# tsy935/eeg-gnn-ssl

Measured on AMD Instinct MI355X. Metric: EEG clips/sec (60s, 19ch, K=2, 2-layer x64) fwd+bwd, higher is better.
Workload: dtype f32

## Files before the change

### eeg_gnn_ssl_amd/csrc/api.cpp

```cpp
#include <atomic>
#include <cmath>
#include <cstdarg>
#include <cstdio>
#include <cstring>

#include <string>
#include <vector>

#include "../../include/eeg_dcrnn.h"
#include "../../include/eeg_dcrnn_dev.h"
#include "../../include/eeg_dcrnn_prof.h"
#include "kernels_decoder.h"
#include "kernels_diffuse.h"
#include "kernels_data.h"
#include "kernels_feat.h"
#include "kernels_gemm.h"
#include "kernels_gemm_bf.h"
#include "kernels_graph.h"
#include "kernels_head.h"
#include "kernels_pack.h"
#include "spec_common.h"
#include "spec_launch.h"
#include "kernels_tail.h"
#include "prof.h"
// ... 555 lines not shown
    if (p == nullptr) return fail("zero: null pointer");
    if (reinterpret_cast<uintptr_t>(p) % 16 != 0)
        return hipMemsetAsync(p, 0, bytes, S_(stream)) == hipSuccess ? 0 : fail("zero: memset failed");
    const size_t n16 = bytes / 16;
    const int blocks = (int)(n16 / 256 < 1 ? 1 : (n16 / 256 > 1024 ? 1024 : n16 / 256));
    EEG_LAUNCH_P("zero", zero_kernel, dim3(blocks), dim3(256), 0, S_(stream), reinterpret_cast<float4*>(p), n16,
                 reinterpret_cast<unsigned char*>(p) + 16 * n16, (int)(bytes - 16 * n16));
    return check_launch("zero");
}

int eeg_dcrnn_hop_polys(const float* const* supports, int n_supports, int n_graphs, int N, int K, float* P_out,
                        void* stream) {
    if (n_supports < 1 || n_supports > 4) return fail("hop_polys: n_supports=%d unsupported (1..4)", n_supports);
    if (N < 1 || N > kMaxNodes) return fail("hop_polys: num_nodes=%d unsupported", N);
    if (K < 0) return fail("hop_polys: max_diffusion_step=%d unsupported (>= 0)", K);
    if (n_graphs < 1) return fail("hop_polys: no graphs (n_graphs=%d)", n_graphs);
    if (K == 0) return 0;
    if (n_supports * K + 1 > kMaxM) return fail("hop_polys: %d supports x K=%d exceeds %d hop matrices", n_supports, K, kMaxM);
    SupPtrs sp;
    for (int i = 0; i < 4; ++i) sp.p[i] = i < n_supports ? supports[i] : nullptr;
    const size_t lds = 4 * kMaxNodes * kMaxNodes * sizeof(float);
    EEG_LAUNCH_P("hop_polys", hop_polys_kernel, dim3(n_graphs), dim3(round_up(N * N, 64)), lds, S_(stream), sp, n_supports, N, K, P_out);
    return check_launch("hop_polys");
}

size_t eeg_dcrnn_pack_floats(int Fin, int H, int M) { return make_cell_pack(Fin, H, M).total; }

int eeg_dcrnn_pack_cell(const float* Wg, const float* bg, const float* Wc, const float* bc, int Fin, int H, int M,
                        float* pack, void* stream) {
    if (!seq_h_supported(H)) return fail("pack_cell: rnn_units=%d unsupported", H);
    if (Fin < 4 || Fin % 4 != 0) return fail("pack_cell: input dim %d must be a positive multiple of 4", Fin);
    if (!seq_m_supported(M)) return fail("pack_cell: num hop matrices M=%d unsupported (1,2,3,4,5,7)", M);
    CellPack p = make_cell_pack(Fin, H, M);
    EEG_LAUNCH_P("pack_cell", pack_cell_kernel, dim3(512), dim3(256), 0, S_(stream), Wg, bg, Wc, bc, pack, p);
    return check_launch("pack_cell");
}
size_t eeg_dcrnn_pack3_halves(int Fin, int H, int M) { return pack3_supported(Fin, H, M) ? make_pack3(Fin, H, M).total : 0; }
int eeg_dcrnn_pack_cell_bf16x3(const float* Wg, const float* Wc, int Fin, int H, int M, uint16_t* pack3, void* stream) {
    if (!pack3_supported(Fin, H, M)) return fail("pack_cell_bf16x3: rnn_units=%d, input_dim=%d, %d hop matrices: the bf16 split exists for 64 units", H, Fin, M);
    if (Wg == nullptr || Wc == nullptr || pack3 == nullptr) return fail("pack_cell_bf16x3: null pointer");
    EEG_LAUNCH_P("pack_cell", pack_cell_bf3_kernel, dim3(512), dim3(256), 0, S_(stream), Wg, Wc, Fin, H, M, pack3);
    return check_launch("pack_cell_bf3");
}

int eeg_dcrnn_diffuse_fwd(const float* X, const float* P, int p_batched, int S, int B, int N, int F, int M,
                          float* planes, void* stream) {
    if (N < 1 || N > kMaxNodes || F < 4 || F % 4 != 0 || M < 1 || M > kMaxM) return fail("diffuse_fwd: bad dims N=%d F=%d M=%d", N, F, M);
    if (S < 1 || B < 1) return fail("diffuse_fwd: empty input (S=%d, B=%d)", S, B);
    return diffuse_fwd(X, P, p_batched, S, B, N, F, M, planes, S_(stream));
}
int eeg_dcrnn_diffuse_adj(const float* Z, const float* P, int p_batched, int S, int B, int N, int F, int M,
                          float* dX, void* stream) {
    if (N < 1 || N > kMaxNodes || F < 4 || F % 4 != 0 || M < 1 || M > kMaxM) return fail("diffuse_adj: bad dims N=%d F=%d M=%d", N, F, M);
    if (S < 1 || B < 1) return fail("diffuse_adj: empty input (S=%d, B=%d)", S, B);
    return diffuse_adj(Z, P, p_batched, S, B, N, F, M, dX, S_(stream));
}

static bool layer_dims_positive(const eeg_layer_dims* d) {
    return d != nullptr && d->T >= 1 && d->B >= 1 && d->N >= 1 && d->H >= 1 && d->Fin >= 1 && d->M >= 1;
}
size_t eeg_dcrnn_layer_fwd_ws_floats(const eeg_layer_dims* d) {
    if (!layer_dims_positive(d)) return 0;
    const size_t xw = (size_t)d->T * d->B * d->N * 3 * d->H;
    return d->spectral != nullptr ? xw + (size_t)d->N * spec_rows(d->T * d->B) * 3 * d->H : xw;
}

size_t eeg_dcrnn_spectral_basis_floats(int N) { return (N >= 1 && N <= kMaxNodes) ? (size_t)spec_basis_floats(N) : 0; }
// ... 1071 lines not shown
```

### eeg_gnn_ssl_amd/csrc/kernels_pack.h

```cpp
#pragma once
#include "common.h"
#include "nnq_order.h"
#include "spec_common.h"
#include "pack_cell.h"

namespace eeg {

__global__ void pack_cell_kernel(const float* __restrict__ Wg, const float* __restrict__ bg,
                                 const float* __restrict__ Wc, const float* __restrict__ bc,
                                 float* __restrict__ out, CellPack p) {
    pack_cell_body(Wg, bg, Wc, bc, out, p, (int)blockIdx.x, (int)gridDim.x);
}

__global__ void pack_dense_kernel(const float* __restrict__ W, int F, int M, int O, float* __restrict__ out) {
    const size_t total = (size_t)F * M * O;
    const int nct = O / 16;
    for (size_t e = (size_t)blockIdx.x * blockDim.x + threadIdx.x; e < total; e += (size_t)gridDim.x * blockDim.x) {
        const int lane = e & 63, ct = (e >> 6) % nct, ks = (e >> 6) / nct;
        const int k = 4 * ks + (lane >> 4), j = 16 * ct + (lane & 15);
        const int m = k / F, f = k % F;
        out[e] = W[((size_t)f * M + m) * O + j];
    }
}

// ... 49 lines not shown
    const float sv[4] = {sum.x, sum.y, sum.z, sum.w};
    const bool accumulate = (kind_flags & 8) != 0;
    const int kind = kind_flags & 7;
#pragma unroll
    for (int e = 0; e < 4; ++e) {
        const size_t idx = idx4 + e;
        const int k = idx / O, o = idx % O;
        float* dst;
        if (kind == 0) {
            const int m = k / Fin, f = k % Fin;
            dst = o < 2 * H ? &dWg[((size_t)f * M + m) * (2 * H) + o] : &dWc[((size_t)f * M + m) * H + (o - 2 * H)];
        } else if (kind == 1) {
            dst = &dWg[((size_t)(Fin + k % H) * M + k / H) * (2 * H) + o];
        } else if (kind == 3) {
            dst = &dWg[idx];
        } else if (kind == 4) {
            dst = &dWg[((size_t)(k % Fin) * M + k / Fin) * O + o];
        } else {
            dst = &dWc[((size_t)(Fin + k % H) * M + k / H) * H + o];
        }
        *dst = accumulate ? *dst + sv[e] : sv[e];
    }
}
__global__ __launch_bounds__(256) void reduce_unpack_kernel(const float* __restrict__ part, int nsplit, int K, int O,
                                                            int kind_flags, int Fin, int H, int M,
                                                            float* __restrict__ dWg, float* __restrict__ dWc) {
    reduce_unpack_block(blockIdx.x, part, nsplit, K, O, kind_flags, Fin, H, M, dWg, dWc);
}
__device__ __forceinline__ void reduce_bias_block(int blk, float* sm, const float* __restrict__ part, int B, int H,
                                                  float* __restrict__ dbg, float* __restrict__ dbc) {
    const int c = threadIdx.x & 15, q = threadIdx.x >> 4;
    const int j = blk * 16 + c;
    float s = 0.f;
    if (j < 3 * H)
        for (int b = q; b < B; b += 16) s += part[(size_t)b * 3 * H + j];
    sm[q * 16 + c] = s;
    __syncthreads();
    if (q == 0 && j < 3 * H) {
        float t = 0.f;
        for (int i = 0; i < 16; ++i) t += sm[i * 16 + c];
        if (j < 2 * H) dbg[j] = t; else dbc[j - 2 * H] = t;
    }
}
struct ReduceJobs {
    const float* part[3]; int nsplit[3]; int K[3]; int O[3]; int nblocks[3];
    const float* bias_part; int bias_B; float* dbg; float* dbc;
};
__global__ __launch_bounds__(256) void reduce_unpack3_kernel(ReduceJobs jobs, int flags, int Fin, int H, int M,
                                                             float* __restrict__ dWg, float* __restrict__ dWc) {
    int b = blockIdx.x, j = 0;
    if (b >= jobs.nblocks[0]) { b -= jobs.nblocks[0]; j = 1; }
    if (j == 1 && b >= jobs.nblocks[1]) { b -= jobs.nblocks[1]; j = 2; }
    if (j == 2 && b >= jobs.nblocks[2]) {
        EEG_DYN_SMEM(sm);
        reduce_bias_block(b - jobs.nblocks[2], sm, jobs.bias_part, jobs.bias_B, H, jobs.dbg, jobs.dbc);
        return;
    }
    reduce_unpack_block(b, jobs.part[j], jobs.nsplit[j], jobs.K[j], jobs.O[j], j | flags, Fin, H, M, dWg, dWc);
}

__global__ __launch_bounds__(256) void reduce_unpack3s_kernel(ReduceJobs jobs, SpecFoldJobs sj, int flags, int Fin, int H, int M,
                                                              float* __restrict__ dWg, float* __restrict__ dWc) {
    int b = blockIdx.x;
#pragma unroll
    for (int k = 0; k < 3; ++k) {
        if (sj.j[k].part == nullptr) continue;
        if (b < sj.j[k].nblocks) {
            spec_fold_block(b, sj.j[k], k, sj.basis, sj.N, (flags & 8) != 0 ? 1 : 0, Fin, H, M, dWg, dWc);
            return;
        }
        b -= sj.j[k].nblocks;
    }
#pragma unroll
    for (int j = 1; j < 3; ++j) {
        if (sj.j[j].part != nullptr) continue;
        if (b < jobs.nblocks[j]) {
            reduce_unpack_block(b, jobs.part[j], jobs.nsplit[j], jobs.K[j], jobs.O[j], j | flags, Fin, H, M, dWg, dWc);
            return;
        }
        b -= jobs.nblocks[j];
    }
    EEG_DYN_SMEM(sm);
    reduce_bias_block(b, sm, jobs.bias_part, jobs.bias_B, H, jobs.dbg, jobs.dbc);
}

__global__ void colsum_partial_kernel(const float* __restrict__ A, int R, int C, int rpc, float* __restrict__ partial) {
    EEG_DYN_SMEM(sm);
    const int c = threadIdx.x & 127, q = threadIdx.x >> 7;
    const int col = blockIdx.y * 128 + c;
    const int r0 = blockIdx.x * rpc, r1 = (r0 + rpc < R) ? r0 + rpc : R;
    float a0 = 0.f, a1 = 0.f, a2 = 0.f, a3 = 0.f;
    if (col < C) {
        int r = r0 + q;
        for (; r + 6 < r1; r += 8) {
// ... 101 lines not shown
```

### eeg_gnn_ssl_amd/csrc/kernels_spectral.h

```cpp
#pragma once
#include "spec_common.h"
#include "spec_launch.h"

namespace eeg {

__global__ __launch_bounds__(256) void spectral_basis_kernel(const float* __restrict__ S, int N, float* __restrict__ out) {
    EEG_DYN_SMEM(sm);
    double* A = reinterpret_cast<double*>(sm);
    double* V = A + 32 * 32;
    double* cs = V + 32 * 32;
    int* pq = reinterpret_cast<int*>(cs + 32);
    double* red = reinterpret_cast<double*>(pq + 32);
    const int tid = threadIdx.x;
    const int NP = (N + 1) & ~1, NH = NP / 2;
    for (int e = tid; e < 32 * 32; e += 256) {
        const int i = e >> 5, j = e & 31;
        A[e] = (i < N && j < N) ? 0.5 * ((double)S[i * N + j] + (double)S[j * N + i]) : 0.0;
        V[e] = i == j ? 1.0 : 0.0;
    }
    __syncthreads();
    for (int sweep = 0; sweep < kSpecSweeps; ++sweep) {
        for (int r = 0; r < NP - 1; ++r) {
            if (tid < NH) {
                int p = tid == 0 ? NP - 1 : (r + tid) % (NP - 1);
                int q = tid == 0 ? r : (r - tid + (NP - 1)) % (NP - 1);
                if (p > q) { const int t = p; p = q; q = t; }
                double c = 1.0, s = 0.0;
                if (q < N) {
                    const double apq = A[p * 32 + q];
                    if (fabs(apq) > 1e-300) {
                        const double theta = (A[q * 32 + q] - A[p * 32 + p]) / (2.0 * apq);
                        const double t = (theta >= 0.0 ? 1.0 : -1.0) / (fabs(theta) + sqrt(theta * theta + 1.0));
                        c = 1.0 / sqrt(t * t + 1.0);
                        s = t * c;
// ... 36 lines not shown
            t = m == 0 ? t0 : t1;
            for (int k = 2; k <= m; ++k) { t = 2.0 * lam * t1 - t0; t0 = t1; t1 = t; }
        }
        out[N * N + e] = (float)t;
    }
    double rmax = 0.0, omax = 0.0, smax = 0.0;
    for (int e = tid; e < N * N; e += 256) {
        const int i = e / N, j = e % N;
        double rec = 0.0;
        for (int k = 0; k < N; ++k) rec += V[i * 32 + k] * A[k * 32 + k] * V[j * 32 + k];
        rmax = fmax(rmax, fabs((double)S[e] - rec));
        if (i != j) omax = fmax(omax, fabs(A[i * 32 + j]));
        smax = fmax(smax, fabs((double)S[e]));
    }
    for (int which = 0; which < 3; ++which) {
        __syncthreads();
        red[tid] = which == 0 ? rmax : (which == 1 ? omax : smax);
        __syncthreads();
        if (tid == 0) {
            double m = 0.0;
            for (int i = 0; i < 256; ++i) m = fmax(m, red[i]);
            out[N * N + kSpecTc + which] = (float)m;
        }
    }
    if (tid >= 3 && tid < kSpecInfo) out[N * N + kSpecTc + tid] = 0.f;
    if (tid < 32) {
        double c = 0.0;
        if (tid < N)
            for (int n = 0; n < N; ++n) c += V[n * 32 + tid];
        out[N * N + kSpecTc + kSpecInfo + tid] = (float)c;
    }
}

__device__ __forceinline__ void pack_spectral_body(const float* __restrict__ Wg, const float* __restrict__ Wc, const float* __restrict__ basis,
                                                   float* __restrict__ out, const SpecPack& p, int bid, int nb) {
    const int Fin = p.Fin, H = p.H, M = p.M, N = p.N;
    const float* tc = basis + N * N;
    const NnqOrder ox = make_nnq_order(1, Fin), ot = make_nnq_order(1, 3 * H);
    const size_t stride = (size_t)nb * blockDim.x;
    for (size_t idx = (size_t)bid * blockDim.x + threadIdx.x; idx < p.total; idx += stride) {
        if (idx >= p.sxr) {
            const size_t e0 = idx - p.sxr;
            const int i = (int)(e0 / p.sxr_stride), e = (int)(e0 - (size_t)i * p.sxr_stride), f = e / (3 * H), o = e - f * 3 * H;
            float v = 0.f;
            if (f < Fin)
                for (int m = 0; m < M; ++m) {
                    const float w = o < 2 * H ? Wg[((size_t)f * M + m) * (2 * H) + o] : Wc[((size_t)f * M + m) * H + (o - 2 * H)];
                    v = fmaf(tc[m * 32 + i], w, v);
                }
            out[idx] = v;
            continue;
        }
        const bool tr = idx >= p.sxtq;
        const size_t bs = tr ? p.sxtq_stride : p.sxq_stride, e0 = idx - (tr ? p.sxtq : p.sxq);
        const int i = (int)(e0 / bs);
        const size_t e = e0 - (size_t)i * bs;
        const int s4 = e & 3, lane = (e >> 2) & 63, nct = tr ? p.nct_t : p.nct_x;
        const int ct = (int)((e >> 8) % nct), c = (int)((e >> 8) / nct), j = 16 * ct + (lane & 15);
        const int k = nnq_k_of(tr ? ot : ox, c, lane >> 4, s4);
        float v = 0.f;
        if (k >= 0) {
            const int f = tr ? j : k, o = tr ? k : j;
            if (f < Fin) {
                for (int m = 0; m < M; ++m) {
                    const float w = o < 2 * H ? Wg[((size_t)f * M + m) * (2 * H) + o] : Wc[((size_t)f * M + m) * H + (o - 2 * H)];
                    v = fmaf(tc[m * 32 + i], w, v);
                }
            }
        }
        out[idx] = v;
    }
}
__global__ void pack_spectral_kernel(const float* __restrict__ Wg, const float* __restrict__ Wc, const float* __restrict__ basis,
                                     float* __restrict__ out, SpecPack p) {
    pack_spectral_body(Wg, Wc, basis, out, p, (int)blockIdx.x, (int)gridDim.x);
}

__device__ __forceinline__ size_t spec_sample(size_t r, int map, int T, int B) { return map ? (r % B) * (size_t)T + r / B : r; }

template <int N>
__global__ __launch_bounds__(256) void spec_mix_in_kernel(const float* __restrict__ X, const float* __restrict__ basis, int S, int Sp,
                                                         int F, int map, int T, int B, float* __restrict__ Xh) {
    const int F4 = F / 4, SPW = blockDim.x / F4;
    const int tl = threadIdx.x / F4, c4 = threadIdx.x % F4;
    if (tl >= SPW) return;
    const float* __restrict__ U = basis;
    const float4* X4 = reinterpret_cast<const float4*>(X);
    float4* O4 = reinterpret_cast<float4*>(Xh);
    for (int r = blockIdx.x * SPW + tl; r < Sp; r += gridDim.x * SPW) {
        if (r >= S) {
#pragma unroll
            for (int i = 0; i < N; ++i) O4[((size_t)i * Sp + r) * F4 + c4] = make_float4(0.f, 0.f, 0.f, 0.f);
            continue;
        }
        const size_t s = spec_sample((size_t)r, map, T, B);
        float4 x[N];
#pragma unroll
        for (int n = 0; n < N; ++n) x[n] = X4[(s * N + n) * F4 + c4];
#pragma unroll
        for (int i = 0; i < N; ++i) {
            float4 a = make_float4(0.f, 0.f, 0.f, 0.f);
#pragma unroll
            for (int n = 0; n < N; ++n) {
// ... 133 lines not shown
```

### eeg_gnn_ssl_amd/csrc/pack_cell.h

```cpp
#pragma once
#include "common.h"
#include "nnq_order.h"

namespace eeg {

struct CellPack {
    int Fin, H, M;
    size_t bx;
    size_t bias;
    size_t bhg;
    size_t bhc;
    size_t b1;
    size_t b2;
    size_t bxt;
    size_t c1;
    size_t c2;
    size_t bxq;
    size_t bxtq;
    bool has_bxq, has_bxtq;
    size_t total;
};

__host__ __device__ inline CellPack make_cell_pack(int Fin, int H, int M) {
    CellPack p;
    p.Fin = Fin; p.H = H; p.M = M;
    size_t o = 0;
    p.bx = o;   o += (size_t)M * Fin * 3 * H;
    p.bias = o; o += (size_t)round_up(3 * H, 64);
    p.bhg = o;  o += (size_t)M * H * 2 * H;
    p.bhc = o;  o += (size_t)M * H * H;
    p.b1 = o;   o += (size_t)M * H * H;
    p.b2 = o;   o += (size_t)M * 2 * H * H;
    p.bxt = o;  o += (size_t)3 * H * round_up(M * Fin, 16);
    p.c1 = o;   o += (size_t)M * H * cell_pack_cx_cols(Fin, H);
    p.c2 = o;   o += (size_t)M * 2 * H * cell_pack_cx_cols(Fin, H);
    p.has_bxq = (3 * H) % 192 == 0;
    p.has_bxtq = (M * Fin) % 192 == 0 && (3 * H) % 4 == 0 && make_nnq_order(1, 3 * H).ntail <= 2;
    p.bxq = o;  o += p.has_bxq ? (size_t)round_up(make_nnq_order(M, Fin).nch, 4) * (3 * H / 16) * 256 : 0;
    p.bxtq = o; o += p.has_bxtq ? (size_t)make_nnq_order(1, 3 * H).nch * (M * Fin / 16) * 256 : 0;
    p.total = o;
    return p;
}

__device__ __forceinline__ float ref_wg(const float* Wg, int M, int H, int f_all, int m, int o) {
    return Wg[((size_t)f_all * M + m) * (2 * H) + o];
}
__device__ __forceinline__ float ref_wc(const float* Wc, int M, int H, int f_all, int m, int o) {
    return Wc[((size_t)f_all * M + m) * H + o];
}

__device__ __forceinline__ void pack_cell_body(const float* __restrict__ Wg, const float* __restrict__ bg,
                                               const float* __restrict__ Wc, const float* __restrict__ bc,
                                               float* __restrict__ out, const CellPack& p, int bid, int nb) {
    const int Fin = p.Fin, H = p.H, M = p.M;
    const size_t stride = (size_t)nb * blockDim.x;
    for (size_t idx = (size_t)bid * blockDim.x + threadIdx.x; idx < p.total; idx += stride) {
        float v = 0.f;
        if (idx < p.bias) {
            const size_t e = idx - p.bx;
            const int lane = e & 63, nct = 3 * H / 16;
            const int ct = (e >> 6) % nct, ks = (e >> 6) / nct;
            const int k = 4 * ks + (lane >> 4), j = 16 * ct + (lane & 15);
            const int m = k / Fin, f = k % Fin;
            v = j < 2 * H ? ref_wg(Wg, M, H, f, m, j) : ref_wc(Wc, M, H, f, m, j - 2 * H);
        } else if (idx < p.bhg) {
            const int j = idx - p.bias;
            v = j < 2 * H ? bg[j] : (j < 3 * H ? bc[j - 2 * H] : 0.f);
        } else if (idx < p.bhc) {
            const size_t e = idx - p.bhg;
            const int lane = e & 63, nct = 2 * H / 16;
            const int ct = (e >> 6) % nct, ks = (e >> 6) / nct;
            const int k = kperm(ks, lane >> 4), j = 16 * ct + (lane & 15);
            v = ref_wg(Wg, M, H, Fin + k % H, k / H, j);
        } else if (idx < p.b1) {
            const size_t e = idx - p.bhc;
            const int lane = e & 63, nct = H / 16;
            const int ct = (e >> 6) % nct, ks = (e >> 6) / nct;
            const int k = kperm(ks, lane >> 4), j = 16 * ct + (lane & 15);
            v = ref_wc(Wc, M, H, Fin + k % H, k / H, j);
        } else if (idx < p.b2) {
            const size_t e = idx - p.b1;
            const int lane = e & 63, nct = H / 16;
            const int ct = (e >> 6) % nct, ks = (e >> 6) / nct;
            const int k = kperm(ks, lane >> 4), f = 16 * ct + (lane & 15);
            v = ref_wc(Wc, M, H, Fin + f, k / H, k % H);
        } else if (idx < p.bxt) {
            const size_t e = idx - p.b2;
            const int lane = e & 63, nct = H / 16;
            const int ct = (e >> 6) % nct, ks = (e >> 6) / nct;
            const int k = kperm(ks, lane >> 4), f = 16 * ct + (lane & 15);
            v = ref_wg(Wg, M, H, Fin + f, k / (2 * H), k % (2 * H));
        } else if (idx < p.c1) {
            const size_t e = idx - p.bxt;
            const int lane = e & 63, nct = round_up(M * Fin, 16) / 16;
            const int ct = (e >> 6) % nct, ks = (e >> 6) / nct;
            const int o = 4 * ks + (lane >> 4), j = 16 * ct + (lane & 15);
            if (j < M * Fin) {
                const int m = j / Fin, f = j % Fin;
                v = o < 2 * H ? ref_wg(Wg, M, H, f, m, o) : ref_wc(Wc, M, H, f, m, o - 2 * H);
            }
        } else if (idx >= p.bxq) {
            const bool tr = idx >= p.bxtq;
            const size_t e = idx - (tr ? p.bxtq : p.bxq);
            const int s4 = e & 3, lane = (e >> 2) & 63, nct = tr ? M * Fin / 16 : 3 * H / 16;
            const int ct = (e >> 8) % nct, c = (e >> 8) / nct, j = 16 * ct + (lane & 15);
            const int k = nnq_k_of(tr ? make_nnq_order(1, 3 * H) : make_nnq_order(M, Fin), c, lane >> 4, s4);
            if (k >= 0) {
                if (!tr) {
                    const int m = k / Fin, f = k % Fin;
                    v = j < 2 * H ? ref_wg(Wg, M, H, f, m, j) : ref_wc(Wc, M, H, f, m, j - 2 * H);
                } else {
                    const int m = j / Fin, f = j % Fin;
                    v = k < 2 * H ? ref_wg(Wg, M, H, f, m, k) : ref_wc(Wc, M, H, f, m, k - 2 * H);
                }
            }
        } else {
            const bool gate = idx >= p.c2;
            const size_t e = idx - (gate ? p.c2 : p.c1);
            const int lane = e & 63, nct = cell_pack_cx_cols(Fin, H) / 16, W = gate ? 2 * H : H;
            const int ct = (e >> 6) % nct, ks = (e >> 6) / nct;
            const int k = kperm(ks, lane >> 4), j = 16 * ct + (lane & 15);
            const int f_all = j < H ? Fin + j : j - H;
            if (j < H + Fin) v = gate ? ref_wg(Wg, M, H, f_all, k / W, k % W) : ref_wc(Wc, M, H, f_all, k / W, k % W);
        }
        out[idx] = v;
    }
}
}
```

### eeg_gnn_ssl_amd/csrc/spec_common.h

```cpp
#pragma once
#include "common.h"
#include "nnq_order.h"

namespace eeg {

constexpr int kSpecTc = kMaxM * 32, kSpecInfo = 32, kSpecCsum = 32;
__host__ __device__ constexpr int spec_basis_floats(int N) { return N * N + kSpecTc + kSpecInfo + kSpecCsum; }
__host__ __device__ constexpr int spec_csum_offset(int N) { return N * N + kSpecTc + kSpecInfo; }
__host__ __device__ constexpr int spec_rows(int S) { return round_up(S, 16); }
constexpr int kSpecSweeps = 12;

struct SpecPack {
    int Fin, H, M, N;
    int nch_x, nct_x, nch_t, nct_t;
    size_t sxq, sxq_stride, sxtq, sxtq_stride, sxr, sxr_stride, total;
};
__host__ __device__ inline SpecPack make_spec_pack(int Fin, int H, int M, int N) {
    SpecPack p;
    p.Fin = Fin; p.H = H; p.M = M; p.N = N;
    p.nch_x = make_nnq_order(1, Fin).nch; p.nct_x = 3 * H / 16;
    p.nch_t = make_nnq_order(1, 3 * H).nch; p.nct_t = round_up(Fin, 16) / 16;
    p.sxq_stride = (size_t)p.nch_x * p.nct_x * 256;
    p.sxtq_stride = (size_t)p.nch_t * p.nct_t * 256;
    p.sxq = 0;
    p.sxtq = p.sxq + p.sxq_stride * N;
    p.sxr = p.sxtq + p.sxtq_stride * N;
    p.sxr_stride = (size_t)round_up(Fin, 8) * 3 * H;
    p.total = p.sxr + p.sxr_stride * N;
    return p;
}
struct SpecFoldJob {
    const float* part;
    int spg, K, O, nblocks;
};
struct SpecFoldJobs {
    SpecFoldJob j[3];
    const float* basis;
    int N;
};
__host__ __device__ inline size_t spec_fold_lds_bytes(int M, int nsplit_max) { return 256 * 16 + (size_t)M * nsplit_max * sizeof(float); }
template <int MM>
__device__ __forceinline__ void spec_fold_block_m(int block, const SpecFoldJob& jb, int kind, const float* __restrict__ basis, int N,
                                                   int acc_flag, int Fin, int H, int M, float* __restrict__ dWg, float* __restrict__ dWc) {
    EEG_DYN_SMEM(sm);
    float4 (*red)[16] = reinterpret_cast<float4 (*)[16]>(sm);
    float* tcl = sm + 256 * 4;
    const int O = jb.O;
    const size_t total = (size_t)jb.K * O;
    const int g = threadIdx.x >> 4, q = threadIdx.x & 15;
    const size_t idx4 = ((size_t)block * 16 + q) * 4;
    const float* tc = basis + N * N;
    const int nsplit = N * jb.spg;
    for (int e = threadIdx.x; e < M * nsplit; e += 256) {
        const int m = e / nsplit, sp = e - m * nsplit;
        tcl[e] = tc[m * 32 + sp / jb.spg];
    }
    __syncthreads();
    float4 a[MM];
#pragma unroll
    for (int m = 0; m < MM; ++m) a[m] = make_float4(0.f, 0.f, 0.f, 0.f);
    if (idx4 < total) {
        constexpr int UN = 8;
        for (int base = g; base < nsplit; base += 16 * UN) {
            float4 v[UN];
#pragma unroll
            for (int u = 0; u < UN; ++u) {
                const int sp = base + 16 * u;
                v[u] = sp < nsplit ? *reinterpret_cast<const float4*>(jb.part + (size_t)sp * total + idx4) : make_float4(0.f, 0.f, 0.f, 0.f);
            }
#pragma unroll
            for (int u = 0; u < UN; ++u) {
                const int sp = base + 16 * u < nsplit ? base + 16 * u : 0;
#pragma unroll
                for (int m = 0; m < MM; ++m) {
                    if (m < M) {
                        const float t = tcl[m * nsplit + sp];
                        a[m].x = fmaf(t, v[u].x, a[m].x); a[m].y = fmaf(t, v[u].y, a[m].y);
                        a[m].z = fmaf(t, v[u].z, a[m].z); a[m].w = fmaf(t, v[u].w, a[m].w);
                    }
                }
            }
        }
    }
#pragma unroll
    for (int m = 0; m < MM; ++m) {
        if (m >= M) break;
        __syncthreads();
        red[g][q] = a[m];
        __syncthreads();
        if (g == 0 && idx4 < total) {
            float4 sum = red[0][q];
#pragma unroll
            for (int u = 1; u < 16; ++u) {
                const float4 v = red[u][q];
                sum.x += v.x; sum.y += v.y; sum.z += v.z; sum.w += v.w;
            }
            const float sv[4] = {sum.x, sum.y, sum.z, sum.w};
#pragma unroll
            for (int e = 0; e < 4; ++e) {
                const size_t idx = idx4 + e;
                const int f = (int)(idx / O), o = (int)(idx % O);
                float* dst;
                if (kind == 0) dst = o < 2 * H ? &dWg[((size_t)f * M + m) * (2 * H) + o] : &dWc[((size_t)f * M + m) * H + (o - 2 * H)];
                else if (kind == 1) dst = &dWg[((size_t)(Fin + f) * M + m) * (2 * H) + o];
                else dst = &dWc[((size_t)(Fin + f) * M + m) * H + o];
                *dst = acc_flag ? *dst + sv[e] : sv[e];
            }
        }
    }
}
__device__ __forceinline__ void spec_fold_block(int block, const SpecFoldJob& jb, int kind, const float* __restrict__ basis, int N,
                                                int acc_flag, int Fin, int H, int M, float* __restrict__ dWg, float* __restrict__ dWc) {
    if (M <= 4) spec_fold_block_m<4>(block, jb, kind, basis, N, acc_flag, Fin, H, M, dWg, dWc);
    else spec_fold_block_m<kMaxM>(block, jb, kind, basis, N, acc_flag, Fin, H, M, dWg, dWc);
}

}
```

### eeg_gnn_ssl_amd/csrc/spec_inst.cpp

```cpp
#include "kernels_gemm_g.h"
#include "kernels_gemm_f.h"
#include "kernels_spectral.h"
#include "pack_cell.h"
#include "spec_launch.h"
#include "prof.h"

namespace eeg {

constexpr int kMaxPackJobs = 8;
struct PackJob {
    const float *Wg, *bg, *Wc, *bc, *basis;
    float* out;
    int spectral;
    CellPack cp;
    SpecPack sp;
};
struct PackJobs { PackJob j[kMaxPackJobs]; };
__global__ void pack_cells_kernel(PackJobs jobs) {
    const PackJob& jb = jobs.j[blockIdx.y];
    if (jb.spectral) pack_spectral_body(jb.Wg, jb.Wc, jb.basis, jb.out, jb.sp, (int)blockIdx.x, (int)gridDim.x);
    else pack_cell_body(jb.Wg, jb.bg, jb.Wc, jb.bc, jb.out, jb.cp, (int)blockIdx.x, (int)gridDim.x);
}


size_t spec_pack_floats(int Fin, int H, int M, int N) { return make_spec_pack(Fin, H, M, N).total; }

int launch_spec_basis(const float* S, int N, float* basis, hipStream_t st) {
    EEG_SET_MAX_LDS(spectral_basis_kernel, kSpecBasisLds);
    EEG_LAUNCH_P("spec_basis", spectral_basis_kernel, dim3(1), dim3(256), kSpecBasisLds, st, S, N, basis);
    return hipGetLastError() == hipSuccess ? 0 : 2;
}

int launch_spec_pack(const float* Wg, const float* Wc, const float* basis, int Fin, int H, int M, int N, float* spack, hipStream_t st) {
    const SpecPack p = make_spec_pack(Fin, H, M, N);
    EEG_LAUNCH_P("pack_cell", pack_spectral_kernel, dim3(1024), dim3(256), 0, st, Wg, Wc, basis, spack, p);
    return hipGetLastError() == hipSuccess ? 0 : 2;
}

int launch_pack_cells(int n_cells, const float* const* Wg, const float* const* bg, const float* const* Wc, const float* const* bc,
                      const int* Fin, int H, int M, float* const* packs, const float* basis, int N, float* const* spacks, hipStream_t st) {
    PackJobs jobs{};
    int n = 0;
    for (int c = 0; c < n_cells; ++c) {
        if (n + (spacks != nullptr ? 2 : 1) > kMaxPackJobs) return 1;
        PackJob& a = jobs.j[n++];
        a.Wg = Wg[c]; a.bg = bg[c]; a.Wc = Wc[c]; a.bc = bc[c]; a.basis = nullptr; a.out = packs[c]; a.spectral = 0;
        a.cp = make_cell_pack(Fin[c], H, M);
        if (spacks != nullptr) {
            PackJob& b = jobs.j[n++];
            b.Wg = Wg[c]; b.bg = nullptr; b.Wc = Wc[c]; b.bc = nullptr; b.basis = basis; b.out = spacks[c]; b.spectral = 1;
            b.sp = make_spec_pack(Fin[c], H, M, N);
        }
    }
    EEG_LAUNCH_P("pack_cell", pack_cells_kernel, dim3(256, n), dim3(256), 0, st, jobs);
    return hipGetLastError() == hipSuccess ? 0 : 2;
}

int launch_spec_mix(const SpecMixPlan& p, const float* in, const float* basis, int N, int T, int B, int F, int bm, float* out,
                    hipStream_t st, const char* tag) {
    const float* bias = nullptr;
    const dim3 grid(p.grid), block(p.block);
#define EEG_MIX_MFMA(DIR, KS) EEG_LAUNCH_P(tag, (spec_mix_mfma_kernel<DIR, KS>), grid, block, p.lds, st, in, basis, bias, N, p.S, p.Sp, F, bm, T, B, out)
    if (p.kind == SpecMixKind::Mfma) {
        if (p.ks == 10) { if (p.to_nodes) EEG_MIX_MFMA(0, 10); else EEG_MIX_MFMA(1, 10); }
        else { if (p.to_nodes) EEG_MIX_MFMA(0, 16); else EEG_MIX_MFMA(1, 16); }
    } else if (p.kind == SpecMixKind::Valu19) {
        if (p.to_nodes) EEG_LAUNCH_P(tag, spec_mix_in_kernel<19>, grid, block, p.lds, st, in, basis, p.S, p.Sp, F, bm, T, B, out);
        else EEG_LAUNCH_P(tag, spec_mix_out_kernel<19>, grid, block, p.lds, st, in, basis, bias, p.S, p.Sp, F, bm, T, B, out);
    } else {
        EEG_LAUNCH_P(tag, spec_mix_generic_kernel, grid, block, p.lds, st, in, basis, bias, N, p.S, p.Sp, F, bm, T, B, p.to_nodes, out);
    }
#undef EEG_MIX_MFMA
    return hipGetLastError() == hipSuccess ? 0 : 2;
}

int launch_spec_zero_rows(float* Xh, int N, int S, int Sp, int F, hipStream_t st) {
    if (Sp <= S) return 0;
    EEG_LAUNCH_P("zero", spec_zero_pad_kernel, dim3(ceil_div(N * (Sp - S) * F, 256)), dim3(256), 0, st, Xh, N, S, Sp, F);
    return hipGetLastError() == hipSuccess ? 0 : 2;
}

namespace {
template <int KQ, bool SWZ>
void launch_nnf_one(const SpecNnPlan& p, const float* A, size_t ags, int K, int Sp, int G, const float* Wr, size_t wstride, float* C, hipStream_t st,
                    const char* tag, const float* bias, const float* gscale) {
    EEG_SET_MAX_LDS((gemm_nnf_kernel<KQ, SWZ>), p.lds);
    EEG_LAUNCH_P(tag, (gemm_nnf_kernel<KQ, SWZ>), dim3(p.grid), dim3(p.block), p.lds, st, A, (long long)ags, K, Sp, G, Wr, (unsigned)wstride, C, bias, gscale);
// ... 101 lines not shown
```

Before: 140,000.

## Vectorize weight packing, size pack grids per job, and pipeline spectral fold reduction

Weight packing kernels now compute four consecutive outputs per thread with 32-bit indices and store them as float4. The spectral pack hoists the per-element weight loads out of the node loop so each weight is reused across all N outputs. Pack grids are sized from each job's float count, with jobs laid out along one flattened grid instead of a fixed 256xn grid. The spectral gradient fold double-buffers its partial-sum loads, reduces all hop matrices through one LDS pass with vector stores, and the bias reduction and fold kernel get unrolling and a launch bound that asks for two blocks per SIMD. This adds index-range checks and uses more LDS in the fold.

```diff
diff --git a/eeg_gnn_ssl_amd/csrc/api.cpp b/eeg_gnn_ssl_amd/csrc/api.cpp
--- a/eeg_gnn_ssl_amd/csrc/api.cpp
+++ b/eeg_gnn_ssl_amd/csrc/api.cpp
@@ -611,7 +611,8 @@
     if (Fin < 4 || Fin % 4 != 0) return fail("pack_cell: input dim %d must be a positive multiple of 4", Fin);
     if (!seq_m_supported(M)) return fail("pack_cell: num hop matrices M=%d unsupported (1,2,3,4,5,7)", M);
     CellPack p = make_cell_pack(Fin, H, M);
-    EEG_LAUNCH_P("pack_cell", pack_cell_kernel, dim3(512), dim3(256), 0, S_(stream), Wg, bg, Wc, bc, pack, p);
+    if (p.total >= kPackIndexLimit) return fail("pack_cell: %zu floats of packs exceed the 32-bit index range", p.total);
+    EEG_LAUNCH_P("pack_cell", pack_cell_kernel, dim3(pack_blocks(p.total)), dim3(256), 0, S_(stream), Wg, bg, Wc, bc, pack, p);
     return check_launch("pack_cell");
 }
 size_t eeg_dcrnn_pack3_halves(int Fin, int H, int M) { return pack3_supported(Fin, H, M) ? make_pack3(Fin, H, M).total : 0; }
diff --git a/eeg_gnn_ssl_amd/csrc/kernels_pack.h b/eeg_gnn_ssl_amd/csrc/kernels_pack.h
--- a/eeg_gnn_ssl_amd/csrc/kernels_pack.h
+++ b/eeg_gnn_ssl_amd/csrc/kernels_pack.h
@@ -105,8 +105,17 @@
     const int c = threadIdx.x & 15, q = threadIdx.x >> 4;
     const int j = blk * 16 + c;
     float s = 0.f;
-    if (j < 3 * H)
-        for (int b = q; b < B; b += 16) s += part[(size_t)b * 3 * H + j];
+    if (j < 3 * H) {
+        constexpr int UN = 8;
+        for (int b0 = q; b0 < B; b0 += 16 * UN) {
+            float v[UN];
+#pragma unroll
+            for (int u = 0; u < UN; ++u) v[u] = b0 + 16 * u < B ? part[(size_t)(b0 + 16 * u) * 3 * H + j] : 0.f;
+#pragma unroll
+            for (int u = 0; u < UN; ++u)
+                if (b0 + 16 * u < B) s += v[u];
+        }
+    }
     sm[q * 16 + c] = s;
     __syncthreads();
     if (q == 0 && j < 3 * H) {
@@ -132,7 +141,7 @@
     reduce_unpack_block(b, jobs.part[j], jobs.nsplit[j], jobs.K[j], jobs.O[j], j | flags, Fin, H, M, dWg, dWc);
 }
 
-__global__ __launch_bounds__(256) void reduce_unpack3s_kernel(ReduceJobs jobs, SpecFoldJobs sj, int flags, int Fin, int H, int M,
+__global__ __launch_bounds__(256, 2) void reduce_unpack3s_kernel(ReduceJobs jobs, SpecFoldJobs sj, int flags, int Fin, int H, int M,
                                                               float* __restrict__ dWg, float* __restrict__ dWc) {
     int b = blockIdx.x;
 #pragma unroll
diff --git a/eeg_gnn_ssl_amd/csrc/kernels_spectral.h b/eeg_gnn_ssl_amd/csrc/kernels_spectral.h
--- a/eeg_gnn_ssl_amd/csrc/kernels_spectral.h
+++ b/eeg_gnn_ssl_amd/csrc/kernels_spectral.h
@@ -1,5 +1,6 @@
 #pragma once
 #include "spec_common.h"
+#include "pack_cell.h"
 #include "spec_launch.h"
 
 namespace eeg {
@@ -102,43 +103,56 @@
     }
 }
 
+__host__ __device__ inline size_t spec_pack_block_floats(const SpecPack& p) { return p.sxq_stride + p.sxtq_stride + p.sxr_stride; }
 __device__ __forceinline__ void pack_spectral_body(const float* __restrict__ Wg, const float* __restrict__ Wc, const float* __restrict__ basis,
                                                    float* __restrict__ out, const SpecPack& p, int bid, int nb) {
     const int Fin = p.Fin, H = p.H, M = p.M, N = p.N;
     const float* tc = basis + N * N;
     const NnqOrder ox = make_nnq_order(1, Fin), ot = make_nnq_order(1, 3 * H);
-    const size_t stride = (size_t)nb * blockDim.x;
-    for (size_t idx = (size_t)bid * blockDim.x + threadIdx.x; idx < p.total; idx += stride) {
-        if (idx >= p.sxr) {
-            const size_t e0 = idx - p.sxr;
-            const int i = (int)(e0 / p.sxr_stride), e = (int)(e0 - (size_t)i * p.sxr_stride), f = e / (3 * H), o = e - f * 3 * H;
-            float v = 0.f;
-            if (f < Fin)
-                for (int m = 0; m < M; ++m) {
-                    const float w = o < 2 * H ? Wg[((size_t)f * M + m) * (2 * H) + o] : Wc[((size_t)f * M + m) * H + (o - 2 * H)];
-                    v = fmaf(tc[m * 32 + i], w, v);
+    const unsigned s0 = (unsigned)p.sxq_stride, s1 = s0 + (unsigned)p.sxtq_stride, total = s1 + (unsigned)p.sxr_stride;
+    const unsigned stride = 4u * (unsigned)nb * blockDim.x;
+    for (unsigned idx = 4u * ((unsigned)bid * blockDim.x + threadIdx.x); idx < total; idx += stride) {
+        float* dst;
+        unsigned bs;
+        int f[4], o[4];
+        if (idx >= s1) {
+            const int e = (int)(idx - s1), r = e / (3 * H), c = e - r * 3 * H;
+#pragma unroll
+            for (int s = 0; s < 4; ++s) { f[s] = r; o[s] = c + s; }
+            dst = out + p.sxr + e; bs = (unsigned)p.sxr_stride;
+        } else {
+            const bool tr = idx >= s0;
+            const unsigned e = idx - (tr ? s0 : 0u);
+            const int lane = (e >> 2) & 63, nct = tr ? p.nct_t : p.nct_x;
+            const int ct = (int)((e >> 8) % nct), c = (int)((e >> 8) / nct), j = 16 * ct + (lane & 15);
+#pragma unroll
+            for (int s = 0; s < 4; ++s) {
+                const int k = nnq_k_of(tr ? ot : ox, c, lane >> 4, s);
+                f[s] = k < 0 ? -1 : (tr ? j : k);
+                o[s] = tr ? k : j;
+            }
+            dst = out + (tr ? p.sxtq : p.sxq) + e; bs = (unsigned)(tr ? p.sxtq_stride : p.sxq_stride);
+        }
+        float w[4][kMaxM];
+#pragma unroll
+        for (int s = 0; s < 4; ++s)
+#pragma unroll
+            for (int m = 0; m < kMaxM; ++m) {
+                w[s][m] = 0.f;
+                if (m < M && f[s] >= 0 && f[s] < Fin)
+                    w[s][m] = o[s] < 2 * H ? Wg[((size_t)f[s] * M + m) * (2 * H) + o[s]] : Wc[((size_t)f[s] * M + m) * H + (o[s] - 2 * H)];
+            }
+        for (int i = 0; i < N; ++i) {
+            f32x4 v = {0.f, 0.f, 0.f, 0.f};
+#pragma unroll
+            for (int m = 0; m < kMaxM; ++m)
+                if (m < M) {
+                    const float t = tc[m * 32 + i];
+#pragma unroll
+                    for (int s = 0; s < 4; ++s) v[s] = fmaf(t, w[s][m], v[s]);
                 }
-            out[idx] = v;
-            continue;
-        }
-        const bool tr = idx >= p.sxtq;
-        const size_t bs = tr ? p.sxtq_stride : p.sxq_stride, e0 = idx - (tr ? p.sxtq : p.sxq);
-        const int i = (int)(e0 / bs);
-        const size_t e = e0 - (size_t)i * bs;
-        const int s4 = e & 3, lane = (e >> 2) & 63, nct = tr ? p.nct_t : p.nct_x;
-        const int ct = (int)((e >> 8) % nct), c = (int)((e >> 8) / nct), j = 16 * ct + (lane & 15);
-        const int k = nnq_k_of(tr ? ot : ox, c, lane >> 4, s4);
-        float v = 0.f;
-        if (k >= 0) {
-            const int f = tr ? j : k, o = tr ? k : j;
-            if (f < Fin) {
-                for (int m = 0; m < M; ++m) {
-                    const float w = o < 2 * H ? Wg[((size_t)f * M + m) * (2 * H) + o] : Wc[((size_t)f * M + m) * H + (o - 2 * H)];
-                    v = fmaf(tc[m * 32 + i], w, v);
-                }
-            }
-        }
-        out[idx] = v;
+            pack_store4(dst + (size_t)i * bs, v);
+        }
     }
 }
 __global__ void pack_spectral_kernel(const float* __restrict__ Wg, const float* __restrict__ Wc, const float* __restrict__ basis,
diff --git a/eeg_gnn_ssl_amd/csrc/pack_cell.h b/eeg_gnn_ssl_amd/csrc/pack_cell.h
--- a/eeg_gnn_ssl_amd/csrc/pack_cell.h
+++ b/eeg_gnn_ssl_amd/csrc/pack_cell.h
@@ -49,81 +49,98 @@
     return Wc[((size_t)f_all * M + m) * H + o];
 }
 
+__device__ __forceinline__ float pack_cell_elem(const float* __restrict__ Wg, const float* __restrict__ bg,
+                                                const float* __restrict__ Wc, const float* __restrict__ bc,
+                                                const CellPack& p, unsigned idx, int s) {
+    const int Fin = p.Fin, H = p.H, M = p.M;
+    float v = 0.f;
+    if (idx < (unsigned)p.bias) {
+        const unsigned e = idx - (unsigned)p.bx;
+        const int lane = (e & 60) + s, nct = 3 * H / 16;
+        const int ct = (e >> 6) % nct, ks = (e >> 6) / nct;
+        const int k = 4 * ks + (lane >> 4), j = 16 * ct + (lane & 15);
+        const int m = k / Fin, f = k % Fin;
+        v = j < 2 * H ? ref_wg(Wg, M, H, f, m, j) : ref_wc(Wc, M, H, f, m, j - 2 * H);
+    } else if (idx < (unsigned)p.bhg) {
+        const int j = idx - (unsigned)p.bias + s;
+        v = j < 2 * H ? bg[j] : (j < 3 * H ? bc[j - 2 * H] : 0.f);
+    } else if (idx < (unsigned)p.bhc) {
+        const unsigned e = idx - (unsigned)p.bhg;
+        const int lane = (e & 60) + s, nct = 2 * H / 16;
+        const int ct = (e >> 6) % nct, ks = (e >> 6) / nct;
+        const int k = kperm(ks, lane >> 4), j = 16 * ct + (lane & 15);
+        v = ref_wg(Wg, M, H, Fin + k % H, k / H, j);
+    } else if (idx < (unsigned)p.b1) {
+        const unsigned e = idx - (unsigned)p.bhc;
+        const int lane = (e & 60) + s, nct = H / 16;
+        const int ct = (e >> 6) % nct, ks = (e >> 6) / nct;
+        const int k = kperm(ks, lane >> 4), j = 16 * ct + (lane & 15);
+        v = ref_wc(Wc, M, H, Fin + k % H, k / H, j);
+    } else if (idx < (unsigned)p.b2) {
+        const unsigned e = idx - (unsigned)p.b1;
+        const int lane = (e & 60) + s, nct = H / 16;
+        const int ct = (e >> 6) % nct, ks = (e >> 6) / nct;
+        const int k = kperm(ks, lane >> 4), f = 16 * ct + (lane & 15);
+        v = ref_wc(Wc, M, H, Fin + f, k / H, k % H);
+    } else if (idx < (unsigned)p.bxt) {
+        const unsigned e = idx - (unsigned)p.b2;
+        const int lane = (e & 60) + s, nct = H / 16;
+        const int ct = (e >> 6) % nct, ks = (e >> 6) / nct;
+        const int k = kperm(ks, lane >> 4), f = 16 * ct + (lane & 15);
+        v = ref_wg(Wg, M, H, Fin + f, k / (2 * H), k % (2 * H));
+    } else if (idx < (unsigned)p.c1) {
+        const unsigned e = idx - (unsigned)p.bxt;
+        const int lane = (e & 60) + s, nct = round_up(M * Fin, 16) / 16;
+        const int ct = (e >> 6) % nct, ks = (e >> 6) / nct;
+        const int o = 4 * ks + (lane >> 4), j = 16 * ct + (lane & 15);
+        if (j < M * Fin) {
+            const int m = j / Fin, f = j % Fin;
+            v = o < 2 * H ? ref_wg(Wg, M, H, f, m, o) : ref_wc(Wc, M, H, f, m, o - 2 * H);
+        }
+    } else if (idx >= (unsigned)p.bxq) {
+        const bool tr = idx >= (unsigned)p.bxtq;
+        const unsigned e = idx - (unsigned)(tr ? p.bxtq : p.bxq);
+        const int s4 = s, lane = (e >> 2) & 63, nct = tr ? M * Fin / 16 : 3 * H / 16;
+        const int ct = (e >> 8) % nct, c = (e >> 8) / nct, j = 16 * ct + (lane & 15);
+        const int k = nnq_k_of(tr ? make_nnq_order(1, 3 * H) : make_nnq_order(M, Fin), c, lane >> 4, s4);
+        if (k >= 0) {
+            if (!tr) {
+                const int m = k / Fin, f = k % Fin;
+                v = j < 2 * H ? ref_wg(Wg, M, H, f, m, j) : ref_wc(Wc, M, H, f, m, j - 2 * H);
+            } else {
+                const int m = j / Fin, f = j % Fin;
+                v = k < 2 * H ? ref_wg(Wg, M, H, f, m, k) : ref_wc(Wc, M, H, f, m, k - 2 * H);
+            }
+        }
+    } else {
+        const bool gate = idx >= (unsigned)p.c2;
+        const unsigned e = idx - (unsigned)(gate ? p.c2 : p.c1);
+        const int lane = (e & 60) + s, nct = cell_pack_cx_cols(Fin, H) / 16, W = gate ? 2 * H : H;
+        const int ct = (e >> 6) % nct, ks = (e >> 6) / nct;
+        const int k = kperm(ks, lane >> 4), j = 16 * ct + (lane & 15);
+        const int f_all = j < H ? Fin + j : j - H;
+        if (j < H + Fin) v = gate ? ref_wg(Wg, M, H, f_all, k / W, k % W) : ref_wc(Wc, M, H, f_all, k / W, k % W);
+    }
+    return v;
+}
+
+constexpr unsigned kPackIndexLimit = 1u << 31;
+__host__ __device__ inline unsigned pack_blocks(size_t total) { return (unsigned)((total / 4 + 255) / 256); }
+
+__device__ __forceinline__ void pack_store4(float* dst, f32x4 v) {
+    if ((reinterpret_cast<size_t>(dst) & 15) == 0) st4(dst, v);
+    else { dst[0] = v[0]; dst[1] = v[1]; dst[2] = v[2]; dst[3] = v[3]; }
+}
+
 __device__ __forceinline__ void pack_cell_body(const float* __restrict__ Wg, const float* __restrict__ bg,
                                                const float* __restrict__ Wc, const float* __restrict__ bc,
                                                float* __restrict__ out, const CellPack& p, int bid, int nb) {
-    const int Fin = p.Fin, H = p.H, M = p.M;
-    const size_t stride = (size_t)nb * blockDim.x;
-    for (size_t idx = (size_t)bid * blockDim.x + threadIdx.x; idx < p.total; idx += stride) {
-        float v = 0.f;
-        if (idx < p.bias) {
-            const size_t e = idx - p.bx;
-            const int lane = e & 63, nct = 3 * H / 16;
-            const int ct = (e >> 6) % nct, ks = (e >> 6) / nct;
-            const int k = 4 * ks + (lane >> 4), j = 16 * ct + (lane & 15);
-            const int m = k / Fin, f = k % Fin;
-            v = j < 2 * H ? ref_wg(Wg, M, H, f, m, j) : ref_wc(Wc, M, H, f, m, j - 2 * H);
-        } else if (idx < p.bhg) {
-            const int j = idx - p.bias;
-            v = j < 2 * H ? bg[j] : (j < 3 * H ? bc[j - 2 * H] : 0.f);
-        } else if (idx < p.bhc) {
-            const size_t e = idx - p.bhg;
-            const int lane = e & 63, nct = 2 * H / 16;
-            const int ct = (e >> 6) % nct, ks = (e >> 6) / nct;
-            const int k = kperm(ks, lane >> 4), j = 16 * ct + (lane & 15);
-            v = ref_wg(Wg, M, H, Fin + k % H, k / H, j);
-        } else if (idx < p.b1) {
-            const size_t e = idx - p.bhc;
-            const int lane = e & 63, nct = H / 16;
-            const int ct = (e >> 6) % nct, ks = (e >> 6) / nct;
-            const int k = kperm(ks, lane >> 4), j = 16 * ct + (lane & 15);
-            v = ref_wc(Wc, M, H, Fin + k % H, k / H, j);
-        } else if (idx < p.b2) {
-            const size_t e = idx - p.b1;
-            const int lane = e & 63, nct = H / 16;
-            const int ct = (e >> 6) % nct, ks = (e >> 6) / nct;
-            const int k = kperm(ks, lane >> 4), f = 16 * ct + (lane & 15);
-            v = ref_wc(Wc, M, H, Fin + f, k / H, k % H);
-        } else if (idx < p.bxt) {
-            const size_t e = idx - p.b2;
-            const int lane = e & 63, nct = H / 16;
-            const int ct = (e >> 6) % nct, ks = (e >> 6) / nct;
-            const int k = kperm(ks, lane >> 4), f = 16 * ct + (lane & 15);
-            v = ref_wg(Wg, M, H, Fin + f, k / (2 * H), k % (2 * H));
-        } else if (idx < p.c1) {
-            const size_t e = idx - p.bxt;
-            const int lane = e & 63, nct = round_up(M * Fin, 16) / 16;
-            const int ct = (e >> 6) % nct, ks = (e >> 6) / nct;
-            const int o = 4 * ks + (lane >> 4), j = 16 * ct + (lane & 15);
-            if (j < M * Fin) {
-                const int m = j / Fin, f = j % Fin;
-                v = o < 2 * H ? ref_wg(Wg, M, H, f, m, o) : ref_wc(Wc, M, H, f, m, o - 2 * H);
-            }
-        } else if (idx >= p.bxq) {
-            const bool tr = idx >= p.bxtq;
-            const size_t e = idx - (tr ? p.bxtq : p.bxq);
-            const int s4 = e & 3, lane = (e >> 2) & 63, nct = tr ? M * Fin / 16 : 3 * H / 16;
-            const int ct = (e >> 8) % nct, c = (e >> 8) / nct, j = 16 * ct + (lane & 15);
-            const int k = nnq_k_of(tr ? make_nnq_order(1, 3 * H) : make_nnq_order(M, Fin), c, lane >> 4, s4);
-            if (k >= 0) {
-                if (!tr) {
-                    const int m = k / Fin, f = k % Fin;
-                    v = j < 2 * H ? ref_wg(Wg, M, H, f, m, j) : ref_wc(Wc, M, H, f, m, j - 2 * H);
-                } else {
-                    const int m = j / Fin, f = j % Fin;
-                    v = k < 2 * H ? ref_wg(Wg, M, H, f, m, k) : ref_wc(Wc, M, H, f, m, k - 2 * H);
-                }
-            }
-        } else {
-            const bool gate = idx >= p.c2;
-            const size_t e = idx - (gate ? p.c2 : p.c1);
-            const int lane = e & 63, nct = cell_pack_cx_cols(Fin, H) / 16, W = gate ? 2 * H : H;
-            const int ct = (e >> 6) % nct, ks = (e >> 6) / nct;
-            const int k = kperm(ks, lane >> 4), j = 16 * ct + (lane & 15);
-            const int f_all = j < H ? Fin + j : j - H;
-            if (j < H + Fin) v = gate ? ref_wg(Wg, M, H, f_all, k / W, k % W) : ref_wc(Wc, M, H, f_all, k / W, k % W);
-        }
-        out[idx] = v;
+    const unsigned total = (unsigned)p.total, stride = 4u * (unsigned)nb * blockDim.x;
+    for (unsigned idx = 4u * ((unsigned)bid * blockDim.x + threadIdx.x); idx < total; idx += stride) {
+        f32x4 v;
+#pragma unroll
+        for (int s = 0; s < 4; ++s) v[s] = pack_cell_elem(Wg, bg, Wc, bc, p, idx, s);
+        pack_store4(out + idx, v);
     }
 }
 }
diff --git a/eeg_gnn_ssl_amd/csrc/spec_common.h b/eeg_gnn_ssl_amd/csrc/spec_common.h
--- a/eeg_gnn_ssl_amd/csrc/spec_common.h
+++ b/eeg_gnn_ssl_amd/csrc/spec_common.h
@@ -38,74 +38,108 @@
     const float* basis;
     int N;
 };
-__host__ __device__ inline size_t spec_fold_lds_bytes(int M, int nsplit_max) { return 256 * 16 + (size_t)M * nsplit_max * sizeof(float); }
+__host__ __device__ inline size_t spec_fold_lds_bytes(int M, int nsplit_max) {
+    return (size_t)M * 256 * 16 + (size_t)round_up(M * nsplit_max, 4) * sizeof(float);
+}
 template <int MM>
 __device__ __forceinline__ void spec_fold_block_m(int block, const SpecFoldJob& jb, int kind, const float* __restrict__ basis, int N,
                                                    int acc_flag, int Fin, int H, int M, float* __restrict__ dWg, float* __restrict__ dWc) {
     EEG_DYN_SMEM(sm);
-    float4 (*red)[16] = reinterpret_cast<float4 (*)[16]>(sm);
-    float* tcl = sm + 256 * 4;
+    const int nsplit = N * jb.spg;
+    float* tcl = sm;
+    float4 (*red)[16][16] = reinterpret_cast<float4 (*)[16][16]>(sm + round_up(M * nsplit, 4));
     const int O = jb.O;
     const size_t total = (size_t)jb.K * O;
     const int g = threadIdx.x >> 4, q = threadIdx.x & 15;
     const size_t idx4 = ((size_t)block * 16 + q) * 4;
     const float* tc = basis + N * N;
-    const int nsplit = N * jb.spg;
-    for (int e = threadIdx.x; e < M * nsplit; e += 256) {
-        const int m = e / nsplit, sp = e - m * nsplit;
-        tcl[e] = tc[m * 32 + sp / jb.spg];
-    }
-    __syncthreads();
+    const bool on = idx4 < total;
+    constexpr int UN = MM <= 4 ? 8 : 4;
+    const float4 zero = make_float4(0.f, 0.f, 0.f, 0.f);
+    const float* src = jb.part + (on ? idx4 : 0);
+    auto request = [&](float4 (&v)[UN], int base0) {
+#pragma unroll
+        for (int u = 0; u < UN; ++u) {
+            const int sp = base0 + g + 16 * u;
+            v[u] = zero;
+            if (base0 + 16 * u < nsplit) {
+                const float4 x = *reinterpret_cast<const float4*>(src + (size_t)(sp < nsplit ? sp : nsplit - 1) * total);
+                if (on && sp < nsplit) v[u] = x;
+            }
+        }
+    };
     float4 a[MM];
 #pragma unroll
-    for (int m = 0; m < MM; ++m) a[m] = make_float4(0.f, 0.f, 0.f, 0.f);
-    if (idx4 < total) {
-        constexpr int UN = 8;
-        for (int base = g; base < nsplit; base += 16 * UN) {
-            float4 v[UN];
+    for (int m = 0; m < MM; ++m) a[m] = zero;
+    auto consume = [&](const float4 (&v)[UN], int base0) {
 #pragma unroll
-            for (int u = 0; u < UN; ++u) {
-                const int sp = base + 16 * u;
-                v[u] = sp < nsplit ? *reinterpret_cast<const float4*>(jb.part + (size_t)sp * total + idx4) : make_float4(0.f, 0.f, 0.f, 0.f);
-            }
+        for (int u = 0; u < UN; ++u) {
+            const int sp = base0 + g + 16 * u < nsplit ? base0 + g + 16 * u : 0;
 #pragma unroll
-            for (int u = 0; u < UN; ++u) {
-                const int sp = base + 16 * u < nsplit ? base + 16 * u : 0;
-#pragma unroll
-                for (int m = 0; m < MM; ++m) {
-                    if (m < M) {
-                        const float t = tcl[m * nsplit + sp];
-                        a[m].x = fmaf(t, v[u].x, a[m].x); a[m].y = fmaf(t, v[u].y, a[m].y);
-                        a[m].z = fmaf(t, v[u].z, a[m].z); a[m].w = fmaf(t, v[u].w, a[m].w);
-                    }
+            for (int m = 0; m < MM; ++m) {
+                if (m < M) {
+                    const float t = tcl[m * nsplit + sp];
+                    a[m].x = fmaf(t, v[u].x, a[m].x); a[m].y = fmaf(t, v[u].y, a[m].y);
+                    a[m].z = fmaf(t, v[u].z, a[m].z); a[m].w = fmaf(t, v[u].w, a[m].w);
                 }
             }
         }
+    };
+    float tv[MM][2];
+#pragma unroll
+    for (int r = 0; r < 2; ++r) {
+        const int sp = threadIdx.x + 256 * r;
+#pragma unroll
+        for (int m = 0; m < MM; ++m) tv[m][r] = (m < M && sp < nsplit) ? tc[m * 32 + sp / jb.spg] : 0.f;
+    }
+    float4 v0[UN], v1[UN];
+    request(v0, 0);
+    request(v1, 16 * UN);
+#pragma unroll
+    for (int r = 0; r < 2; ++r) {
+        const int sp = threadIdx.x + 256 * r;
+#pragma unroll
+        for (int m = 0; m < MM; ++m)
+            if (m < M && sp < nsplit) tcl[m * nsplit + sp] = tv[m][r];
+    }
+    for (int sp = threadIdx.x + 512; sp < nsplit; sp += 256)
+        for (int m = 0; m < M; ++m) tcl[m * nsplit + sp] = tc[m * 32 + sp / jb.spg];
+    __syncthreads();
+#pragma unroll 1
+    for (int base0 = 0; base0 < nsplit; base0 += 32 * UN) {
+        consume(v0, base0);
+        request(v0, base0 + 32 * UN);
+        consume(v1, base0 + 16 * UN);
+        request(v1, base0 + 48 * UN);
     }
 #pragma unroll
-    for (int m = 0; m < MM; ++m) {
-        if (m >= M) break;
-        __syncthreads();
-        red[g][q] = a[m];
-        __syncthreads();
-        if (g == 0 && idx4 < total) {
-            float4 sum = red[0][q];
+    for (int m = 0; m < MM; ++m)
+        if (m < M) red[m][g][q] = a[m];
+    __syncthreads();
+    for (int m = g; m < M; m += 16) {
+        if (!on) break;
+        float4 sum = red[m][0][q];
 #pragma unroll
-            for (int u = 1; u < 16; ++u) {
-                const float4 v = red[u][q];
-                sum.x += v.x; sum.y += v.y; sum.z += v.z; sum.w += v.w;
+        for (int u = 1; u < 16; ++u) {
+            const float4 v = red[m][u][q];
+            sum.x += v.x; sum.y += v.y; sum.z += v.z; sum.w += v.w;
+        }
+        const int f = (int)(idx4 / O), o = (int)(idx4 % O);
+        float* dst;
+        if (kind == 0) dst = o < 2 * H ? &dWg[((size_t)f * M + m) * (2 * H) + o] : &dWc[((size_t)f * M + m) * H + (o - 2 * H)];
+        else if (kind == 1) dst = &dWg[((size_t)(Fin + f) * M + m) * (2 * H) + o];
+        else dst = &dWc[((size_t)(Fin + f) * M + m) * H + o];
+        if ((reinterpret_cast<size_t>(dst) & 15) == 0) {
+            float4 r = sum;
+            if (acc_flag) {
+                const float4 old = *reinterpret_cast<const float4*>(dst);
+                r.x = old.x + sum.x; r.y = old.y + sum.y; r.z = old.z + sum.z; r.w = old.w + sum.w;
             }
+            *reinterpret_cast<float4*>(dst) = r;
+        } else {
             const float sv[4] = {sum.x, sum.y, sum.z, sum.w};
 #pragma unroll
-            for (int e = 0; e < 4; ++e) {
-                const size_t idx = idx4 + e;
-                const int f = (int)(idx / O), o = (int)(idx % O);
-                float* dst;
-                if (kind == 0) dst = o < 2 * H ? &dWg[((size_t)f * M + m) * (2 * H) + o] : &dWc[((size_t)f * M + m) * H + (o - 2 * H)];
-                else if (kind == 1) dst = &dWg[((size_t)(Fin + f) * M + m) * (2 * H) + o];
-                else dst = &dWc[((size_t)(Fin + f) * M + m) * H + o];
-                *dst = acc_flag ? *dst + sv[e] : sv[e];
-            }
+            for (int e = 0; e < 4; ++e) dst[e] = acc_flag ? dst[e] + sv[e] : sv[e];
         }
     }
 }
diff --git a/eeg_gnn_ssl_amd/csrc/spec_inst.cpp b/eeg_gnn_ssl_amd/csrc/spec_inst.cpp
--- a/eeg_gnn_ssl_amd/csrc/spec_inst.cpp
+++ b/eeg_gnn_ssl_amd/csrc/spec_inst.cpp
@@ -12,14 +12,18 @@
     const float *Wg, *bg, *Wc, *bc, *basis;
     float* out;
     int spectral;
+    unsigned first, nb;
     CellPack cp;
     SpecPack sp;
 };
 struct PackJobs { PackJob j[kMaxPackJobs]; };
-__global__ void pack_cells_kernel(PackJobs jobs) {
-    const PackJob& jb = jobs.j[blockIdx.y];
-    if (jb.spectral) pack_spectral_body(jb.Wg, jb.Wc, jb.basis, jb.out, jb.sp, (int)blockIdx.x, (int)gridDim.x);
-    else pack_cell_body(jb.Wg, jb.bg, jb.Wc, jb.bc, jb.out, jb.cp, (int)blockIdx.x, (int)gridDim.x);
+__global__ void pack_cells_kernel(PackJobs jobs, int n) {
+    int k = 0;
+    while (k + 1 < n && blockIdx.x >= jobs.j[k + 1].first) ++k;
+    const PackJob& jb = jobs.j[k];
+    const int bid = (int)(blockIdx.x - jb.first), nb = (int)jb.nb;
+    if (jb.spectral) pack_spectral_body(jb.Wg, jb.Wc, jb.basis, jb.out, jb.sp, bid, nb);
+    else pack_cell_body(jb.Wg, jb.bg, jb.Wc, jb.bc, jb.out, jb.cp, bid, nb);
 }
 
 
@@ -33,7 +37,8 @@
 
 int launch_spec_pack(const float* Wg, const float* Wc, const float* basis, int Fin, int H, int M, int N, float* spack, hipStream_t st) {
     const SpecPack p = make_spec_pack(Fin, H, M, N);
-    EEG_LAUNCH_P("pack_cell", pack_spectral_kernel, dim3(1024), dim3(256), 0, st, Wg, Wc, basis, spack, p);
+    if (p.total >= kPackIndexLimit) return 1;
+    EEG_LAUNCH_P("pack_cell", pack_spectral_kernel, dim3(pack_blocks(spec_pack_block_floats(p))), dim3(256), 0, st, Wg, Wc, basis, spack, p);
     return hipGetLastError() == hipSuccess ? 0 : 2;
 }
 
@@ -41,18 +46,26 @@
                       const int* Fin, int H, int M, float* const* packs, const float* basis, int N, float* const* spacks, hipStream_t st) {
     PackJobs jobs{};
     int n = 0;
+    unsigned nblocks = 0;
+    auto place = [&](PackJob& j, size_t total) {
+        j.first = nblocks; j.nb = pack_blocks(total);
+        nblocks += j.nb;
+        return total < kPackIndexLimit;
+    };
     for (int c = 0; c < n_cells; ++c) {
         if (n + (spacks != nullptr ? 2 : 1) > kMaxPackJobs) return 1;
         PackJob& a = jobs.j[n++];
         a.Wg = Wg[c]; a.bg = bg[c]; a.Wc = Wc[c]; a.bc = bc[c]; a.basis = nullptr; a.out = packs[c]; a.spectral = 0;
         a.cp = make_cell_pack(Fin[c], H, M);
+        if (!place(a, a.cp.total)) return 1;
         if (spacks != nullptr) {
             PackJob& b = jobs.j[n++];
             b.Wg = Wg[c]; b.bg = nullptr; b.Wc = Wc[c]; b.bc = nullptr; b.basis = basis; b.out = spacks[c]; b.spectral = 1;
             b.sp = make_spec_pack(Fin[c], H, M, N);
+            if (b.sp.total >= kPackIndexLimit || !place(b, spec_pack_block_floats(b.sp))) return 1;
         }
     }
-    EEG_LAUNCH_P("pack_cell", pack_cells_kernel, dim3(256, n), dim3(256), 0, st, jobs);
+    EEG_LAUNCH_P("pack_cell", pack_cells_kernel, dim3(nblocks), dim3(256), 0, st, jobs, n);
     return hipGetLastError() == hipSuccess ? 0 : 2;
 }
 
```

New measurement: 140,700 (median of 6 runs). About the same (+0.5%).
